# privefl/bigsnpr

Measured on NVIDIA H100. Metric: genotypes/sec in bed_prodVec, higher is better.
Workload: dtype f64

## Files before the change

bigsnpr_b200/csrc/bsg_pmv.cu:

```cuda
#include <algorithm>
#include <math.h>
#include <stdio.h>
#include <stdlib.h>
#include <string.h>

#include <cub/device/device_scan.cuh>

#include "bsg_internal.cuh"
#include "bsg_pmv_shared.cuh"

namespace bsg {
namespace pmv {

constexpr int SEG = 128;
constexpr int CODES = 512;
constexpr int DIG = 4096;
constexpr int STAGES = 6;
constexpr int STAGE_BYTES = 2 * DIG;
constexpr int SMEM_BYTES = STAGES * STAGE_BYTES + 128;
constexpr int MAX_CHUNKS_PER_ITEM = 512;

struct Args {
  const uint8_t *P;
  int64_t stride;
  const int *lines;
  int nlines;
  int nlines_pad;
  int nchunks;
  int chunks_per_split;
  int ksplit;
  const uint8_t *dig1;
  const uint8_t *dig2;
  const uint8_t *na_flags;
  int use_na;
  long long *part;
};

struct Slot {
  uint4 alo, ahi, blo, bhi;
};

__device__ __forceinline__ void slot_load(Slot &s, const uint8_t *pa, const uint8_t *pb, int64_t off) {
  s.alo = ldg_stream(pa + off);
  s.ahi = ldg_stream(pa + off + 64);
  s.blo = ldg_stream(pb + off);
  s.bhi = ldg_stream(pb + off + 64);
}

template <int MODE>
__device__ __forceinline__ uint32_t plane2(uint32_t x) {
  return MODE == 3 ? (x >> 1) : (x & (x >> 1));
}

template <int MODE, bool PRE>
__device__ __forceinline__ void chunk_mma(const Slot &t0, const Slot &t1, uint32_t dig_addr, int (&acc1)[2][4],
                                          int (&acc16)[2][4], int (&accn1)[2][4], int (&accn16)[2][4]) {
  const uint32_t wA0[8] = {t0.alo.x, t0.alo.y, t0.alo.z, t0.alo.w, t0.ahi.x, t0.ahi.y, t0.ahi.z, t0.ahi.w};
  const uint32_t wB0[8] = {t0.blo.x, t0.blo.y, t0.blo.z, t0.blo.w, t0.bhi.x, t0.bhi.y, t0.bhi.z, t0.bhi.w};
  const uint32_t wA1[8] = {t1.alo.x, t1.alo.y, t1.alo.z, t1.alo.w, t1.ahi.x, t1.ahi.y, t1.ahi.z, t1.ahi.w};
  const uint32_t wB1[8] = {t1.blo.x, t1.blo.y, t1.blo.z, t1.blo.w, t1.bhi.x, t1.bhi.y, t1.bhi.z, t1.bhi.w};
  uint4 dpre[8];
  if (PRE) {
#pragma unroll
    for (int w = 0; w < 8; w++) dpre[w] = lds128(dig_addr + w * 512);
  }
#pragma unroll
  for (int w = 0; w < 8; w++) {
    const uint4 d = PRE ? dpre[w] : lds128(dig_addr + w * 512);
    const uint32_t a0 = wA0[w], b0 = wB0[w], a1 = wA1[w], b1 = wB1[w];
    const uint32_t a0t = a0 >> 2, b0t = b0 >> 2, a1t = a1 >> 2, b1t = b1 >> 2;
    mma_u8s8(acc1[0], a0 & 0x03030303u, b0 & 0x03030303u, a0t & 0x03030303u, b0t & 0x03030303u, d.x, d.y);
    mma_u8s8(acc1[1], a1 & 0x03030303u, b1 & 0x03030303u, a1t & 0x03030303u, b1t & 0x03030303u, d.x, d.y);
    mma_u8s8(acc16[0], a0 & 0x30303030u, b0 & 0x30303030u, a0t & 0x30303030u, b0t & 0x30303030u, d.z, d.w);
    mma_u8s8(acc16[1], a1 & 0x30303030u, b1 & 0x30303030u, a1t & 0x30303030u, b1t & 0x30303030u, d.z, d.w);
    if (MODE != 0) {
      uint4 dn = d;
      if (MODE >= 2) dn = lds128(dig_addr + DIG + w * 512);
      const uint32_t a0n = plane2<MODE>(a0), b0n = plane2<MODE>(b0), a0nt = plane2<MODE>(a0t), b0nt = plane2<MODE>(b0t);
      const uint32_t a1n = plane2<MODE>(a1), b1n = plane2<MODE>(b1), a1nt = plane2<MODE>(a1t), b1nt = plane2<MODE>(b1t);
      mma_u8s8(accn1[0], a0n & 0x01010101u, b0n & 0x01010101u, a0nt & 0x01010101u, b0nt & 0x01010101u, dn.x, dn.y);
      mma_u8s8(accn1[1], a1n & 0x01010101u, b1n & 0x01010101u, a1nt & 0x01010101u, b1nt & 0x01010101u, dn.x, dn.y);
      mma_u8s8(accn16[0], a0n & 0x10101010u, b0n & 0x10101010u, a0nt & 0x10101010u, b0nt & 0x10101010u, dn.z, dn.w);
      mma_u8s8(accn16[1], a1n & 0x10101010u, b1n & 0x10101010u, a1nt & 0x10101010u, b1nt & 0x10101010u, dn.z, dn.w);
    }
  }
}

template <int MODE>
__device__ __forceinline__ void tile_mma(const Slot &sl, const uint4 (&b1)[8], uint32_t dig2_addr, int (&acc1)[4],
                                         int (&acc16)[4], int (&accn1)[4], int (&accn16)[4]) {
  const uint32_t wA[8] = {sl.alo.x, sl.alo.y, sl.alo.z, sl.alo.w, sl.ahi.x, sl.ahi.y, sl.ahi.z, sl.ahi.w};
  const uint32_t wB[8] = {sl.blo.x, sl.blo.y, sl.blo.z, sl.blo.w, sl.bhi.x, sl.bhi.y, sl.bhi.z, sl.bhi.w};
#pragma unroll
  for (int w = 0; w < 8; w++) {
    const uint32_t a = wA[w], bq = wB[w];
    const uint32_t at = a >> 2, bt = bq >> 2;
    mma_u8s8(acc1, a & 0x03030303u, bq & 0x03030303u, at & 0x03030303u, bt & 0x03030303u, b1[w].x, b1[w].y);
    mma_u8s8(acc16, a & 0x30303030u, bq & 0x30303030u, at & 0x30303030u, bt & 0x30303030u, b1[w].z, b1[w].w);
    if (MODE != 0) {
      uint4 d = b1[w];
      if (MODE >= 2) d = lds128(dig2_addr + w * 512);
      const uint32_t an = plane2<MODE>(a), bn = plane2<MODE>(bq);
      const uint32_t ant = plane2<MODE>(at), bnt = plane2<MODE>(bt);
      mma_u8s8(accn1, an & 0x01010101u, bn & 0x01010101u, ant & 0x01010101u, bnt & 0x01010101u, d.x, d.y);
      mma_u8s8(accn16, an & 0x10101010u, bn & 0x10101010u, ant & 0x10101010u, bnt & 0x10101010u, d.z, d.w);
    }
  }
}

template <int MODE, int CW, int R, int STRUCT>
__global__ void __launch_bounds__((CW + 1) * 32, 1) k_pmv(const Args a) {
  constexpr int GROUP = CW * 32;
  extern __shared__ __align__(128) uint8_t smem[];
  const int warp = threadIdx.x >> 5, lane = threadIdx.x & 31;
  const uint32_t smem_base = smem_u32(smem);
  const uint32_t bar_base = smem_base + STAGES * STAGE_BYTES;

  if (threadIdx.x == 0) {
    for (int s = 0; s < STAGES; s++) {
      mbar_init(bar_base + 8 * s, 1);
      mbar_init(bar_base + 8 * (STAGES + s), CW);
    }
    asm volatile("fence.mbarrier_init.release.cluster;" ::: "memory");
  }
  __syncthreads();

  const int ngroups = a.nlines_pad / GROUP;
  const int nitems = ngroups * a.ksplit;
  constexpr bool two_dig = MODE >= 2;
  const uint32_t stage_tx = DIG + (two_dig ? DIG : 0);

  int stage = 0;
  uint32_t phase = 0;

  if (warp == CW) {
    if (lane == 0) {
      for (int item = blockIdx.x; item < nitems; item += gridDim.x) {
        const int group = item / a.ksplit, ks = item - group * a.ksplit;
        const int c0 = ks * a.chunks_per_split;
        const int c1 = min(a.nchunks, c0 + a.chunks_per_split);
        for (int c = c0; c < c1; c++) {
          const uint32_t full = bar_base + 8 * stage, empty = bar_base + 8 * (STAGES + stage);
          mbar_wait(empty, phase ^ 1);
          mbar_expect_tx(full, stage_tx);
          const uint32_t dst = smem_base + stage * STAGE_BYTES;
          bulk_g2s(dst, a.dig1 + (int64_t)c * DIG, DIG, full);
          if (two_dig) bulk_g2s(dst + DIG, a.dig2 + (int64_t)c * DIG, DIG, full);
          if (++stage == STAGES) {
            stage = 0;
            phase ^= 1;
          }
        }
      }
    }
  } else {
    const int g = lane >> 2, q = lane & 3;
    for (int item = blockIdx.x; item < nitems; item += gridDim.x) {
      const int group = item / a.ksplit, ks = item - group * a.ksplit;
      const int c0 = ks * a.chunks_per_split;
      const int c1 = min(a.nchunks, c0 + a.chunks_per_split);
      const uint8_t *pA[2], *pB[2];
#pragma unroll
      for (int u = 0; u < 2; u++) {
        int la = min(group * GROUP + warp * 32 + u * 16 + g, a.nlines - 1);
        int lb = min(group * GROUP + warp * 32 + u * 16 + g + 8, a.nlines - 1);
        const int pa = a.lines ? a.lines[la] : la, pb = a.lines ? a.lines[lb] : lb;
        pA[u] = a.P + (int64_t)pa * a.stride + 16 * q;
        pB[u] = a.P + (int64_t)pb * a.stride + 16 * q;
      }
      bool tile_na = false;
      if (MODE == 3) {
        tile_na = true;
      } else if (MODE != 0) {
        if (a.na_flags) {
          int l = min(group * GROUP + warp * 32 + lane, a.nlines - 1);
          const int phys = a.lines ? a.lines[l] : l;
          tile_na = __any_sync(0xffffffffu, a.na_flags[phys] != 0);
        } else {
          tile_na = true;
        }
      }
      int acc1[2][4], acc16[2][4], accn1[2][4], accn16[2][4];
#pragma unroll
      for (int u = 0; u < 2; u++)
#pragma unroll
        for (int k = 0; k < 4; k++) acc1[u][k] = acc16[u][k] = accn1[u][k] = accn16[u][k] = 0;

      Slot ring[R][2];
#pragma unroll
      for (int k = 0; k < R; k++) {
        ring[k][0] = ring[k][1] =
            Slot{make_uint4(0, 0, 0, 0), make_uint4(0, 0, 0, 0), make_uint4(0, 0, 0, 0), make_uint4(0, 0, 0, 0)};
        if (c0 + k < c1) {
          slot_load(ring[k][0], pA[0], pB[0], (int64_t)(c0 + k) * SEG);
          slot_load(ring[k][1], pA[1], pB[1], (int64_t)(c0 + k) * SEG);
        }
      }

      for (int c = c0; c < c1; c += R) {
#pragma unroll
        for (int par = 0; par < R; par++) {
          if (par > 0 && c + par >= c1) break;
          const uint32_t full = bar_base + 8 * stage, empty = bar_base + 8 * (STAGES + stage);
          mbar_wait(full, phase);
          const uint32_t dbase = smem_base + stage * STAGE_BYTES + (g * 4 + q) * 16;
          const int64_t next = (int64_t)(c + par + R) * SEG;
          const bool more = (c + par + R) < c1;
          if (STRUCT == 0) {
            uint4 b1[8];
#pragma unroll
            for (int w = 0; w < 8; w++) b1[w] = lds128(dbase + w * 512);
#pragma unroll
            for (int u = 0; u < 2; u++) {
              if (MODE != 0 && tile_na)
                tile_mma<MODE>(ring[par][u], b1, dbase + DIG, acc1[u], acc16[u], accn1[u], accn16[u]);
              else
                tile_mma<0>(ring[par][u], b1, 0, acc1[u], acc16[u], accn1[u], accn16[u]);
              if (more) slot_load(ring[par][u], pA[u], pB[u], next);
            }
          } else {
            if (MODE != 0 && tile_na)
              chunk_mma<MODE, STRUCT == 2>(ring[par][0], ring[par][1], dbase, acc1, acc16, accn1, accn16);
            else
              chunk_mma<0, STRUCT == 2>(ring[par][0], ring[par][1], dbase, acc1, acc16, accn1, accn16);
            if (more) {
              slot_load(ring[par][0], pA[0], pB[0], next);
              slot_load(ring[par][1], pA[1], pB[1], next);
            }
          }
          __syncwarp();
          if (lane == 0) mbar_arrive(empty);
          if (++stage == STAGES) {
            stage = 0;
            phase ^= 1;
          }
        }
      }
#pragma unroll
      for (int u = 0; u < 2; u++) {
#pragma unroll
        for (int hrow = 0; hrow < 2; hrow++) {
          const int row = group * GROUP + warp * 32 + u * 16 + g + 8 * hrow;
          unsigned long long *dst = reinterpret_cast<unsigned long long *>(a.part) + (int64_t)row * 16 + 2 * q;
          long long vx = (long long)acc1[u][2 * hrow] + (long long)(acc16[u][2 * hrow] >> 4);
          long long vy = (long long)acc1[u][2 * hrow + 1] + (long long)(acc16[u][2 * hrow + 1] >> 4);
          atomicAdd(dst, (unsigned long long)vx);
          atomicAdd(dst + 1, (unsigned long long)vy);
          if (MODE != 0) {
            long long nx = (long long)accn1[u][2 * hrow] + (long long)(accn16[u][2 * hrow] >> 4);
            long long ny = (long long)accn1[u][2 * hrow + 1] + (long long)(accn16[u][2 * hrow + 1] >> 4);
            atomicAdd(dst + 8, (unsigned long long)nx);
            atomicAdd(dst + 9, (unsigned long long)ny);
          }
        }
      }
    }
  }
}


__device__ __forceinline__ void make_vals(int mode, const double *x, const double *center, const double *scale, int k,
                                          double &v0, double &v1) {
  if (mode == 0) {
    v0 = x[k];
    v1 = 0;
  } else if (mode == 2) {
    v0 = x[k];
    v1 = center[k];
  } else {
    double z = x[k] / scale[k];
    v0 = z;
    v1 = (center[k] - 3.0) * z;
  }
}

__global__ void k_prep1(int mode, const double *__restrict__ x, const double *__restrict__ center,
                        const double *__restrict__ scale, int len, int hb, Scal *sc) {
  __shared__ double sh[32];
  double m0 = 0, m1 = 0, cz = 0;
  int bad = 0;
  for (int k = blockIdx.x * blockDim.x + threadIdx.x; k < len; k += gridDim.x * blockDim.x) {
    double v0, v1;
    make_vals(mode, x, center, scale, k, v0, v1);
    if (!isfinite(v0) || !isfinite(v1)) bad = 1;
    m0 = fmax(m0, fabs(v0));
    m1 = fmax(m1, fabs(v1));
    if (mode == 1) cz += center[k] * v0;
  }
#pragma unroll
  for (int o = 16; o; o >>= 1) {
    m0 = fmax(m0, __shfl_xor_sync(0xffffffffu, m0, o));
    m1 = fmax(m1, __shfl_xor_sync(0xffffffffu, m1, o));
    bad |= __shfl_xor_sync(0xffffffffu, bad, o);
    cz += __shfl_xor_sync(0xffffffffu, cz, o);
  }
  if ((threadIdx.x & 31) == 0) {
    atomicMax(reinterpret_cast<unsigned long long *>(&sc->maxabs[0]), (unsigned long long)__double_as_longlong(m0));
    atomicMax(reinterpret_cast<unsigned long long *>(&sc->maxabs[1]), (unsigned long long)__double_as_longlong(m1));
    if (bad) atomicOr(&sc->nonfinite, 1);
    sh[threadIdx.x >> 5] = cz;
  }
  __syncthreads();
  if (threadIdx.x == 0) {
    double t = 0;
    for (int w = 0; w < (int)(blockDim.x >> 5); w++) t += sh[w];
    sc->cpart[blockIdx.x] = t;
    if (blockIdx.x == 0) sc->hb = hb;
  }
}

__global__ void k_quantise(int mode, const double *__restrict__ x, const double *__restrict__ center,
                           const double *__restrict__ scale, int len, const int *__restrict__ idx, const Scal *sc, int bits,
                           long long *__restrict__ Q0, long long *__restrict__ Q1) {
  const int e0 = pick_e(sc->maxabs[0], sc->hb, bits), e1 = pick_e(sc->maxabs[1], sc->hb, bits);
  const bool bad = sc->nonfinite != 0;
  for (int k = blockIdx.x * blockDim.x + threadIdx.x; k < len; k += gridDim.x * blockDim.x) {
    double v0, v1;
    make_vals(mode, x, center, scale, k, v0, v1);
    const long long q0 = bad ? 0 : __double2ll_rn(scalbn(v0, e0));
    const int t = idx ? idx[k] : k;
    atomicAdd(reinterpret_cast<unsigned long long *>(Q0 + t), (unsigned long long)q0);
    if (Q1) {
      const long long q1 = bad ? 0 : __double2ll_rn(scalbn(v1, e1));
      atomicAdd(reinterpret_cast<unsigned long long *>(Q1 + t), (unsigned long long)q1);
    }
  }
}

template <int NV>
__global__ void k_prep2(int mode, const double *__restrict__ x, const double *__restrict__ center,
                        const double *__restrict__ scale, const double *__restrict__ xb, int len, int nchunks, Scal *sc,
                        const long long *__restrict__ Q0, const long long *__restrict__ Q1, uint8_t *__restrict__ dig1,
                        uint8_t *__restrict__ dig2, int want_sum, long long *__restrict__ qout) {
  constexpr int NS = 8 / NV, BITS = NV == 1 ? 60 : 30;
  const Scal &sa = sc[0], &sb = sc[NV - 1];
  const int ea = pick_e(sa.maxabs[0], sa.hb, BITS), eb = pick_e(sb.maxabs[NV == 1 ? 1 : 0], sb.hb, BITS);
  const bool bada = sa.nonfinite != 0, badb = sb.nonfinite != 0;
  if (blockIdx.x == 0 && threadIdx.x == 0) {
    for (int v = 0; v < NV; v++) {
      sc[v].e[0] = pick_e(sc[v].maxabs[0], sc[v].hb, BITS);
      sc[v].e[1] = pick_e(sc[v].maxabs[1], sc[v].hb, BITS);
    }
  }
  long long hi = 0, lo = 0;
  const bool fasta = ea > -1000 && ea < 1000, fastb = eb > -1000 && eb < 1000;
  const double fa = fasta ? scalbn(1.0, ea) : 0.0, fb = fastb ? scalbn(1.0, eb) : 0.0;
  int64_t total = (int64_t)nchunks * 32;
  for (int64_t t = blockIdx.x * (int64_t)blockDim.x + threadIdx.x; t < total; t += (int64_t)gridDim.x * blockDim.x) {
    const int chunk = (int)(t >> 5), wq = (int)(t & 31);
    const int q = wq & 3, w = wq >> 2;
    uint32_t o1[8][4], o2[8][4];
#pragma unroll
    for (int sl = 0; sl < 8; sl++)
#pragma unroll
      for (int c = 0; c < 4; c++) o1[sl][c] = o2[sl][c] = 0;
#pragma unroll
    for (int c = 0; c < 4; c++) {
#pragma unroll
      for (int r = 0; r < 4; r++) {
        int64_t k = (int64_t)chunk * CODES + (w < 4 ? 64 * q + 16 * w : 256 + 64 * q + 16 * (w - 4)) + 4 * r + c;
        long long qa = 0, qb = 0;
        if (k < len) {
          if (Q0) {
            qa = Q0[k];
            if (Q1) qb = Q1[k];
          } else {
            double v0, v1;
            if (!bada) {
              make_vals(mode, x, center, scale, (int)k, v0, v1);
              qa = __double2ll_rn(fasta ? v0 * fa : scalbn(v0, ea));
              if (NV == 1 && dig2) qb = __double2ll_rn(fastb ? v1 * fb : scalbn(v1, eb));
            }
            if (NV == 2 && xb && !badb) {
              make_vals(mode, xb, center, scale, (int)k, v0, v1);
              qb = __double2ll_rn(fastb ? v0 * fb : scalbn(v0, eb));
            }
          }
        }
        if (want_sum) {
          hi += qa >> 32;
          lo += (long long)(unsigned int)(qa & 0xFFFFFFFFll);
        }
        if (qout && k < len) qout[k] = qa;
#pragma unroll
        for (int sl = 0; sl < NS; sl++) {
          o1[sl][c] |= (uint32_t)(peel(qa) & 0xFF) << (8 * r);
          if (NV == 2)
            o1[NS + sl][c] |= (uint32_t)(peel(qb) & 0xFF) << (8 * r);
          else if (dig2)
            o2[sl][c] |= (uint32_t)(peel(qb) & 0xFF) << (8 * r);
        }
      }
    }
#pragma unroll
    for (int sl = 0; sl < 8; sl++) {
      const int64_t unit = (int64_t)chunk * 256 + (w * 8 + sl) * 4 + q;
      reinterpret_cast<uint4 *>(dig1)[unit] = make_uint4(o1[sl][0], o1[sl][1], o1[sl][2], o1[sl][3]);
      if (NV == 1 && dig2) reinterpret_cast<uint4 *>(dig2)[unit] = make_uint4(o2[sl][0], o2[sl][1], o2[sl][2], o2[sl][3]);
    }
  }
  if (want_sum) {
#pragma unroll
    for (int o = 16; o; o >>= 1) {
      hi += __shfl_xor_sync(0xffffffffu, hi, o);
      lo += __shfl_xor_sync(0xffffffffu, lo, o);
    }
    if ((threadIdx.x & 31) == 0 && (hi | lo)) {
      atomicAdd(reinterpret_cast<unsigned long long *>(&sc->sum_hi), (unsigned long long)hi);
      atomicAdd(reinterpret_cast<unsigned long long *>(&sc->sum_lo), (unsigned long long)lo);
    }
  }
}

__global__ void k_finish_cprod(const long long *__restrict__ part, int nlines, const Scal *sc,
                               const double *__restrict__ center, const double *__restrict__ scale, int use_na,
                               double *__restrict__ out) {
  int j = blockIdx.x * blockDim.x + threadIdx.x;
  if (j >= nlines) return;
  if (sc->nonfinite) {
    out[j] = nan("");
    return;
  }
  const int e = sc->e[0];
  double G = combine<8>(part, j, 0, 1, use_na ? -3 : 0, e);
  double N = use_na ? combine<8>(part, j, 0, 0, 1, e) : 0.0;
  if (center) {
    const double Y = scalbn((double)sc->sum_hi, 32 - e) + scalbn((double)sc->sum_lo, -e);
    out[j] = (G - center[j] * (Y - N)) / scale[j];
  } else {
    out[j] = G;
  }
}

__global__ void k_finish_prod(const long long *__restrict__ part, int nlines, const Scal *sc, int has_scaling, int use_na,
                              double *__restrict__ full) {
  int l = blockIdx.x * blockDim.x + threadIdx.x;
  if (l >= nlines) return;
  full[l] = finish_prod_value(part, l, sc, has_scaling, use_na);
}

__global__ void k_finish_planes(const long long *__restrict__ part, int nlines, const Scal *sc, int have_p, int p_same,
                                double cR, double cP, double add0, double *__restrict__ full, double cRb, double cPb,
                                double *__restrict__ fullB) {
  int l = blockIdx.x * blockDim.x + threadIdx.x;
  if (l >= nlines) return;
  if (sc->nonfinite) {
    full[l] = nan("");
    if (fullB) fullB[l] = nan("");
    return;
  }
  const double R = combine<8>(part, l, 0, 1, 0, sc->e[0]);
  const double P = have_p ? combine<8>(part, l, 0, 0, 1, sc->e[p_same ? 0 : 1]) : 0.0;
  full[l] = (cR * R + cP * P) + add0;
  if (fullB) fullB[l] = cRb * R + cPb * P;
}

__global__ void k_gather(const double *__restrict__ full, const int *__restrict__ idx, int len, double *__restrict__ out) {
  int i = blockIdx.x * blockDim.x + threadIdx.x;
  if (i < len) out[i] = full[idx[i]];
}

constexpr int EV_POOL = 128;
static cudaEvent_t g_ev0[EV_POOL], g_ev1[EV_POOL];
static bool g_ev_ready = false;
static bool g_timing = false;
static int g_ev_n = 0;

static int launch_cap(int64_t work, int block, int cap) {
  int64_t g = (work + block - 1) / block;
  if (g < 1) g = 1;
  if (g > cap) g = cap;
  return (int)g;
}

static int launch_cap_pub_impl(int64_t work) { return launch_cap(work, 256, 132 * 16); }

static int hb_bits(int maxmult) {
  int b = 0;
  while ((1 << b) < maxmult) b++;
  return b >= 8 ? b + 1 : b;
}

static int prep_pmv(bsg_view *v, int dir, int mode, const double *x, const double *p1, const double *p2, int nv,
                    const double *xb, bool two, bool want_sum, bool keep_q, cudaStream_t s) {
  bsg_bed *h = v->h;
  const bool cols = dir == 0;
  const int L = cols ? h->m : h->n, len = cols ? v->nc : v->nr;
  const int *idx = (cols ? v->col_identity : v->row_identity) ? nullptr : (cols ? v->d_col : v->d_row);
  const int hb = hb_bits(cols ? v->col_maxmult : v->row_maxmult);
  const int nchunks = (int)((cols ? h->strideB : h->strideA) / SEG);
  Scal *sc = v->s_scal.as<Scal>();
  BSG_TRY(v->s_dig1.ensure((size_t)nchunks * DIG));
  if (two) BSG_TRY(v->s_dig2.ensure((size_t)nchunks * DIG));
  uint8_t *dig1 = v->s_dig1.as<uint8_t>(), *dig2 = two ? v->s_dig2.as<uint8_t>() : nullptr;
  long long *Q0 = nullptr, *Q1 = nullptr;
  if (idx || keep_q) {
    BSG_TRY(v->s_q0.ensure((size_t)L * sizeof(long long)));
    Q0 = v->s_q0.as<long long>();
  }
  if (idx && (two || xb)) {
    BSG_TRY(v->s_q1.ensure((size_t)L * sizeof(long long)));
    Q1 = v->s_q1.as<long long>();
  }
  BSG_CUDA(cudaMemsetAsync(sc, 0, nv * sizeof(Scal), s));
  k_prep1<<<SUMCZ_BLOCKS, 256, 0, s>>>(mode, x, p1, p2, len, hb, sc);
  if (xb) k_prep1<<<SUMCZ_BLOCKS, 256, 0, s>>>(mode, xb, p1, p2, len, hb, sc + 1);
  count_launch(xb ? 2 : 1);
  if (idx) {
    const int bits = nv == 1 ? 60 : 30;
    BSG_CUDA(cudaMemsetAsync(Q0, 0, (size_t)L * sizeof(long long), s));
    if (Q1) BSG_CUDA(cudaMemsetAsync(Q1, 0, (size_t)L * sizeof(long long), s));
    k_quantise<<<launch_cap(len, 256, 592), 256, 0, s>>>(mode, x, p1, p2, len, idx, sc, bits, Q0, nv == 1 ? Q1 : nullptr);
    if (xb) k_quantise<<<launch_cap(len, 256, 592), 256, 0, s>>>(mode, xb, p1, p2, len, idx, sc + 1, bits, Q1, nullptr);
    count_launch(xb ? 2 : 1);
  }
  const int grid = launch_cap((int64_t)nchunks * 32, 128, 1184);
  const long long *src0 = idx ? Q0 : nullptr;
  if (nv == 1)
    k_prep2<1><<<grid, 128, 0, s>>>(mode, x, p1, p2, nullptr, L, nchunks, sc, src0, Q1, dig1, dig2, want_sum,
                                    idx ? nullptr : Q0);
  else
    k_prep2<2><<<grid, 128, 0, s>>>(mode, x, p1, p2, xb, L, nchunks, sc, src0, Q1, dig1, nullptr, want_sum, nullptr);
  count_launch();
  return BSG_OK;
}

static int run_pmv(bsg_view *v, const uint8_t *P, int64_t stride, int L, const int *lines, int nlines,
                   const uint8_t *dig1, const uint8_t *dig2, const uint8_t *na_flags, int use_na, Args *out_args,
                   cudaStream_t s, bool plane_hi = false) {
  static int var_cw = 0, var_r = 0, var_s = 0;
  if (!var_cw) {
    var_cw = 11;
    var_r = 3;
    var_s = 1;
    const char *ev = getenv("BSG_PMV_VARIANT");
    int cw = 0, r = 0, st = 0;
    if (ev && sscanf(ev, "%dx%ds%d", &cw, &r, &st) >= 2) {
      if ((cw == 11 || cw == 15) && (r == 2 || r == 3) && st >= 0 && st <= 2) {
        var_cw = cw;
        var_r = r;
        var_s = st;
      }
    }
  }
  const int GROUP = var_cw * 32;
  Args a;
  a.P = P;
  a.stride = stride;
  a.lines = lines;
  a.nlines = nlines;
  a.nlines_pad = (int)round_up(nlines, GROUP);
  a.nchunks = (int)(round_up(((int64_t)L + 3) / 4, SEG) / SEG);
  int ngroups = a.nlines_pad / GROUP;
  int target_items = 24 * 132;
  int ks = (target_items + ngroups - 1) / ngroups;
  int ks_max = std::max(1, a.nchunks / 16);
  int ks_min = (a.nchunks + MAX_CHUNKS_PER_ITEM - 1) / MAX_CHUNKS_PER_ITEM;
  ks = std::min(ks, ks_max);
  ks = std::max(ks, ks_min);
  ks = std::max(ks, 1);
  a.chunks_per_split = (a.nchunks + ks - 1) / ks;
  a.ksplit = (a.nchunks + a.chunks_per_split - 1) / a.chunks_per_split;
  a.dig1 = dig1;
  a.dig2 = dig2;
  a.na_flags = na_flags;
  a.use_na = use_na;
  BSG_TRY(v->s_part.ensure((size_t)a.nlines_pad * 16 * sizeof(long long)));
  a.part = v->s_part.as<long long>();
  BSG_CUDA(cudaMemsetAsync(a.part, 0, (size_t)a.nlines_pad * 16 * sizeof(long long), s));
  const int mode = plane_hi ? 3 : (!use_na ? 0 : (dig2 ? 2 : 1));
  if (plane_hi && !dig2) return fail(BSG_ERR_ARG, "high-bit plane needs its own digits");
  void (*kern)(const Args) = nullptr;
#define PMV_PICK(CWv, Rv, Sv)                                                                   \
  if (var_cw == CWv && var_r == Rv && var_s == Sv)                                              \
    kern = mode == 0 ? k_pmv<0, CWv, Rv, Sv>                                                    \
                     : (mode == 1 ? k_pmv<1, CWv, Rv, Sv> : (mode == 2 ? k_pmv<2, CWv, Rv, Sv> : k_pmv<3, CWv, Rv, Sv>));
  PMV_PICK(11, 2, 0)
  PMV_PICK(11, 2, 1)
  PMV_PICK(11, 2, 2)
  PMV_PICK(11, 3, 0)
  PMV_PICK(11, 3, 1)
  PMV_PICK(15, 2, 1)
#undef PMV_PICK
  if (!kern) return fail(BSG_ERR_ARG, "unknown k_pmv variant");
  BSG_CUDA(cudaFuncSetAttribute(kern, cudaFuncAttributeMaxDynamicSharedMemorySize, SMEM_BYTES));
  int nsm = 132;
  cudaDeviceGetAttribute(&nsm, cudaDevAttrMultiProcessorCount, v->h->device);
  int nitems = ngroups * a.ksplit;
  int grid = std::min(nitems, nsm);
  if (g_timing) cudaEventRecord(g_ev0[g_ev_n % EV_POOL], s);
  kern<<<grid, (var_cw + 1) * 32, SMEM_BYTES, s>>>(a);
  if (g_timing) {
    cudaEventRecord(g_ev1[g_ev_n % EV_POOL], s);
    g_ev_n++;
  }
  count_launch();
  BSG_CUDA(cudaGetLastError());
  *out_args = a;
  return BSG_OK;
}

}

namespace pmvt {
using namespace pmv;
constexpr int TLINES = 32, TBYTES = 512, TWARPS = 8, TSTAGES = 6;
constexpr int WSTAGE_BYTES = TLINES * 64;
constexpr int TSMEM = TWARPS * TSTAGES * WSTAGE_BYTES;
constexpr int MAX_LINES_PER_ITEM = 1 << 16;

struct TArgs {
  const uint8_t *P;
  int64_t stride;
  const int *lines;
  int nlines;
  const uint8_t *dig;
  int lines_per_split, ksplit, nblocks, n;
  long long *part;
};

__device__ __forceinline__ void cp_async16(uint32_t dst, const void *src, int src_bytes) {
  asm volatile("cp.async.cg.shared.global [%0], [%1], 16, %2;" ::"r"(dst), "l"(src), "r"(src_bytes) : "memory");
}

template <int PLANE>
__global__ void __launch_bounds__(TWARPS * 32, 2) k_pmvT_lines(const TArgs a) {
  extern __shared__ __align__(128) uint8_t smem[];
  const int tid = threadIdx.x, warp = tid >> 5, lane = tid & 31, g = lane >> 2, q = lane & 3;
  const int blk = blockIdx.x % a.nblocks, ks = blockIdx.x / a.nblocks;
  const int64_t byte0 = (int64_t)blk * TBYTES + 64 * warp;
  const int l0 = ks * a.lines_per_split, l1 = min(a.nlines, l0 + a.lines_per_split);
  const int nsteps = (l1 - l0 + TLINES - 1) / TLINES;
  const uint32_t wbase = smem_u32(smem) + warp * (TSTAGES * WSTAGE_BYTES);

  const int lrow = lane >> 2, lch = lane & 3;
  const int64_t colb = (byte0 + 16 * lch < a.stride) ? byte0 + 16 * lch : 0;
  uint32_t dst_off[4];
#pragma unroll
  for (int i = 0; i < 4; i++) {
    const int row = 8 * i + lrow;
    const int hf = row >> 4, qq = (row >> 2) & 3, r = row & 3, sl = lch >> 1, hc = lch & 1;
    dst_off[i] = (uint32_t)((((((r * 2 + hf) * 2 + sl) * 4 + qq) * 8) + 4 * hc) * 4);
  }
  auto issue = [&](int step, int stage) {
    const uint32_t dst = wbase + stage * WSTAGE_BYTES;
#pragma unroll
    for (int i = 0; i < 4; i++) {
      const int t = min(l0 + step * TLINES + 8 * i + lrow, l1 - 1);
      const int phys = a.lines[t];
      cp_async16(dst + dst_off[i], a.P + colb + (int64_t)phys * a.stride, 16);
    }
  };

  int acc[4][4][4];
#pragma unroll
  for (int j = 0; j < 4; j++)
#pragma unroll
    for (int c = 0; c < 4; c++)
#pragma unroll
      for (int k = 0; k < 4; k++) acc[j][c][k] = 0;

#pragma unroll
  for (int st = 0; st < TSTAGES - 1; st++) {
    if (st < nsteps) issue(st, st);
    asm volatile("cp.async.commit_group;" ::: "memory");
  }
  const uint8_t *dg = a.dig + (int64_t)(l0 / TLINES) * 256 + g * 32 + 4 * q;
  uint32_t nb0 = 0, nb1 = 0;
  if (nsteps > 0) {
    nb0 = *reinterpret_cast<const uint32_t *>(dg);
    nb1 = *reinterpret_cast<const uint32_t *>(dg + 16);
  }
  const uint32_t rd_base = wbase + (uint32_t)((q * 8 + g) * 4);

  auto compute = [&](uint32_t st_base, uint32_t b0, uint32_t b1) {
    uint32_t W[2][2][4];
#pragma unroll
    for (int sl = 0; sl < 2; sl++)
#pragma unroll
      for (int hf = 0; hf < 2; hf++) {
        const uint32_t ad = st_base + (hf * 2 + sl) * 128;
        const uint32_t x0 = lds32(ad), x1 = lds32(ad + 512), x2 = lds32(ad + 1024), x3 = lds32(ad + 1536);
        const uint32_t t0 = prmt(x0, x1, 0x5140), t1 = prmt(x2, x3, 0x5140);
        const uint32_t t2 = prmt(x0, x1, 0x7362), t3 = prmt(x2, x3, 0x7362);
        W[sl][hf][0] = prmt(t0, t1, 0x5410);
        W[sl][hf][1] = prmt(t0, t1, 0x7632);
        W[sl][hf][2] = prmt(t2, t3, 0x5410);
        W[sl][hf][3] = prmt(t2, t3, 0x7632);
      }
#pragma unroll
    for (int j = 0; j < 4; j++) {
      uint32_t wa = W[0][0][j], wb = W[1][0][j], wc2 = W[0][1][j], wd = W[1][1][j];
      if (PLANE == 1) {
        wa = wa & (wa >> 1) & 0x55555555u;
        wb = wb & (wb >> 1) & 0x55555555u;
        wc2 = wc2 & (wc2 >> 1) & 0x55555555u;
        wd = wd & (wd >> 1) & 0x55555555u;
      } else if (PLANE == 2) {
        wa = (wa >> 1) & 0x55555555u;
        wb = (wb >> 1) & 0x55555555u;
        wc2 = (wc2 >> 1) & 0x55555555u;
        wd = (wd >> 1) & 0x55555555u;
      }
      mma_u8s8(acc[j][0], wa & 0x03030303u, wb & 0x03030303u, wc2 & 0x03030303u, wd & 0x03030303u, b0, b1);
      mma_u8s8(acc[j][1], wa & 0x0C0C0C0Cu, wb & 0x0C0C0C0Cu, wc2 & 0x0C0C0C0Cu, wd & 0x0C0C0C0Cu, b0, b1);
      mma_u8s8(acc[j][2], wa & 0x30303030u, wb & 0x30303030u, wc2 & 0x30303030u, wd & 0x30303030u, b0, b1);
      mma_u8s8(acc[j][3], wa & 0xC0C0C0C0u, wb & 0xC0C0C0C0u, wc2 & 0xC0C0C0C0u, wd & 0xC0C0C0C0u, b0, b1);
    }
  };

  uint32_t rd_stage = 0, wr_stage = (TSTAGES - 1) * WSTAGE_BYTES;
  const uint8_t *dgn = dg + 256;
  for (int step = 0; step < nsteps; step++) {
    asm volatile("cp.async.wait_group %0;" ::"n"(TSTAGES - 2) : "memory");
    __syncwarp();
    {
      const int nxt = step + TSTAGES - 1;
      if (nxt < nsteps) issue(nxt, (int)(wr_stage / WSTAGE_BYTES));
      asm volatile("cp.async.commit_group;" ::: "memory");
    }
    const uint32_t b0 = nb0, b1 = nb1;
    if (step + 1 < nsteps) {
      nb0 = *reinterpret_cast<const uint32_t *>(dgn);
      nb1 = *reinterpret_cast<const uint32_t *>(dgn + 16);
      dgn += 256;
    }
    compute(rd_base + rd_stage, b0, b1);
    rd_stage = rd_stage + WSTAGE_BYTES == TSTAGES * WSTAGE_BYTES ? 0 : rd_stage + WSTAGE_BYTES;
    wr_stage = wr_stage + WSTAGE_BYTES == TSTAGES * WSTAGE_BYTES ? 0 : wr_stage + WSTAGE_BYTES;
  }
  asm volatile("cp.async.wait_group 0;" ::: "memory");
#pragma unroll
  for (int j = 0; j < 4; j++)
#pragma unroll
    for (int c = 0; c < 4; c++)
#pragma unroll
      for (int sl = 0; sl < 2; sl++) {
        const int64_t sample = 4 * (byte0 + 4 * (8 * sl + g) + j) + c;
        if (sample < a.n) {
          unsigned long long *dst = reinterpret_cast<unsigned long long *>(a.part) + sample * 16 + (PLANE ? 8 : 0) + 2 * q;
          long long v0 = acc[j][c][2 * sl], v1 = acc[j][c][2 * sl + 1];
          v0 >>= 2 * c;
          v1 >>= 2 * c;
          if (v0) atomicAdd(dst, (unsigned long long)v0);
          if (v1) atomicAdd(dst + 1, (unsigned long long)v1);
        }
      }
}

constexpr int TBOX = 32 * 128;
constexpr int TDIG_OFF = 4 * TBOX;
constexpr int TSTAGE_BYTES = 4 * TBOX + 1024;
constexpr int TCSTAGES = 6;
constexpr int TSMEM_TMA = TCSTAGES * TSTAGE_BYTES + 2 * TCSTAGES * 8 + 1024;


template <int PLANE>
__global__ void __launch_bounds__(TWARPS * 32, 2) k_pmvT(const __grid_constant__ CUtensorMap map, const TArgs a) {
  extern __shared__ __align__(128) uint8_t smem[];
  const int tid = threadIdx.x, warp = tid >> 5, lane = tid & 31, g = lane >> 2, q = lane & 3;
  const int blk = blockIdx.x % a.nblocks, ks = blockIdx.x / a.nblocks;
  const int l0 = ks * a.lines_per_split, l1 = min(a.nlines, l0 + a.lines_per_split);
  const int nsteps = (l1 - l0 + TLINES - 1) / TLINES;
  const uint32_t sbase = (smem_u32(smem) + 1023u) & ~1023u;
  const uint32_t bar_base = sbase + TCSTAGES * TSTAGE_BYTES;
  auto fill = [&](int step, int st) {
    const uint32_t full = bar_base + 8 * st, dst = sbase + st * TSTAGE_BYTES;
    const uint8_t *dg = a.dig + (int64_t)(l0 / TLINES + step) * 256;
    mbar_expect_tx(full, 4 * TBOX + 256);
#pragma unroll
    for (int j = 0; j < 4; j++) tma_load_2d(dst + j * TBOX, &map, full, blk * TBYTES + 128 * j, l0 + step * TLINES);
    bulk_g2s(dst + TDIG_OFF, dg, 128, full);
    bulk_g2s(dst + TDIG_OFF + 144, dg + 128, 128, full);
  };
  if (tid == 0) {
    for (int st = 0; st < TCSTAGES; st++) {
      mbar_init(bar_base + 8 * st, 1);
      mbar_init(bar_base + 8 * (TCSTAGES + st), TWARPS);
    }
    asm volatile("fence.mbarrier_init.release.cluster;" ::: "memory");
    for (int st = 0; st < min(TCSTAGES, nsteps); st++) fill(st, st);
  }
  __syncthreads();
  int stage = 0, pstage = 0;
  uint32_t phase = 0, pphase = 0;

  const int64_t byte0 = (int64_t)blk * TBYTES + 64 * warp;
  const int rsw = 2 * (q >> 1);
  const uint32_t chunk0 = (4 * (warp & 1) + (g >> 2)) ^ (4 * (q & 1) + rsw);
  const uint32_t rd_base = sbase + (warp >> 1) * TBOX + q * 512 + (rsw << 7) + chunk0 * 16 + 4 * (g & 3);
  const uint32_t dg_base = sbase + TDIG_OFF + g * 32 + 16 * (g >> 2) + 4 * q;
  const uint32_t sel_lo = rsw ? 0x1054u : 0x5410u, sel_hi = rsw ? 0x3276u : 0x7632u;

  int acc[4][4][4];
#pragma unroll
  for (int j = 0; j < 4; j++)
#pragma unroll
    for (int c = 0; c < 4; c++)
#pragma unroll
      for (int k = 0; k < 4; k++) acc[j][c][k] = 0;

  for (int step = 0; step < nsteps; step++) {
    const uint32_t full = bar_base + 8 * stage, empty = bar_base + 8 * (TCSTAGES + stage);
    const uint32_t so = stage * TSTAGE_BYTES;
    const int cstage = stage;
    const uint32_t cphase = phase;
    mbar_wait(full, phase);
    const uint32_t b0 = lds32(dg_base + so), b1 = lds32(dg_base + so + 16);
    uint32_t W[2][2][4];
#pragma unroll
    for (int sl = 0; sl < 2; sl++)
#pragma unroll
      for (int hf = 0; hf < 2; hf++) {
        const uint32_t ad = rd_base + so, hb = hf * (16 * 128);
        const uint32_t x0 = lds32((ad ^ TRD(0, sl)) + hb), x1 = lds32((ad ^ TRD(1, sl)) + hb);
        const uint32_t x2 = lds32((ad ^ TRD(2, sl)) + hb), x3 = lds32((ad ^ TRD(3, sl)) + hb);
        const uint32_t t0 = prmt(x0, x1, 0x5140), t1 = prmt(x2, x3, 0x5140);
        const uint32_t t2 = prmt(x0, x1, 0x7362), t3 = prmt(x2, x3, 0x7362);
        W[sl][hf][0] = prmt(t0, t1, sel_lo);
        W[sl][hf][1] = prmt(t0, t1, sel_hi);
        W[sl][hf][2] = prmt(t2, t3, sel_lo);
        W[sl][hf][3] = prmt(t2, t3, sel_hi);
      }
    __syncwarp();
    if (lane == 0) mbar_arrive(empty);
    if (++stage == TCSTAGES) {
      stage = 0;
      phase ^= 1;
    }
#pragma unroll
    for (int j = 0; j < 4; j++) {
      uint32_t wa = W[0][0][j], wb = W[1][0][j], wc2 = W[0][1][j], wd = W[1][1][j];
      if (PLANE == 1) {
        wa = wa & (wa >> 1) & 0x55555555u;
        wb = wb & (wb >> 1) & 0x55555555u;
        wc2 = wc2 & (wc2 >> 1) & 0x55555555u;
        wd = wd & (wd >> 1) & 0x55555555u;
      } else if (PLANE == 2) {
        wa = (wa >> 1) & 0x55555555u;
        wb = (wb >> 1) & 0x55555555u;
        wc2 = (wc2 >> 1) & 0x55555555u;
        wd = (wd >> 1) & 0x55555555u;
      }
      mma_u8s8(acc[j][0], wa & 0x03030303u, wb & 0x03030303u, wc2 & 0x03030303u, wd & 0x03030303u, b0, b1);
      mma_u8s8(acc[j][1], wa & 0x0C0C0C0Cu, wb & 0x0C0C0C0Cu, wc2 & 0x0C0C0C0Cu, wd & 0x0C0C0C0Cu, b0, b1);
      mma_u8s8(acc[j][2], wa & 0x30303030u, wb & 0x30303030u, wc2 & 0x30303030u, wd & 0x30303030u, b0, b1);
      mma_u8s8(acc[j][3], wa & 0xC0C0C0C0u, wb & 0xC0C0C0C0u, wc2 & 0xC0C0C0C0u, wd & 0xC0C0C0C0u, b0, b1);
    }
    if (tid == 0 && step >= 1 && step - 1 + TCSTAGES < nsteps) {
      mbar_wait(bar_base + 8 * (TCSTAGES + pstage), pphase);
      fill(step - 1 + TCSTAGES, pstage);
    }
    __syncwarp();
    pstage = cstage;
    pphase = cphase;
  }
#pragma unroll
  for (int j = 0; j < 4; j++)
#pragma unroll
    for (int c = 0; c < 4; c++)
#pragma unroll
      for (int sl = 0; sl < 2; sl++) {
        const int64_t sample = 4 * (byte0 + 4 * (8 * sl + g) + j) + c;
        if (sample < a.n) {
          unsigned long long *dst = reinterpret_cast<unsigned long long *>(a.part) + sample * 16 + (PLANE ? 8 : 0) + 2 * q;
          long long v0 = acc[j][c][2 * sl], v1 = acc[j][c][2 * sl + 1];
          v0 >>= 2 * c;
          v1 >>= 2 * c;
          if (v0) atomicAdd(dst, (unsigned long long)v0);
          if (v1) atomicAdd(dst + 1, (unsigned long long)v1);
        }
      }
}

constexpr int W2STAGE_BYTES = TLINES * 32;
constexpr int T2BYTES = TWARPS * 32;
constexpr int T2SMEM = TWARPS * TSTAGES * W2STAGE_BYTES;

template <int PL, bool LINES>
__global__ void __launch_bounds__(TWARPS * 32, 2) k_pmvT2(const TArgs a, const uint8_t *__restrict__ dig2) {
  extern __shared__ __align__(128) uint8_t smem[];
  const int tid = threadIdx.x, warp = tid >> 5, lane = tid & 31, g = lane >> 2, q = lane & 3;
  const int blk = blockIdx.x % a.nblocks, ks = blockIdx.x / a.nblocks;
  const int64_t byte0 = (int64_t)blk * T2BYTES + 32 * warp;
  const int l0 = ks * a.lines_per_split, l1 = min(a.nlines, l0 + a.lines_per_split);
  const int nsteps = (l1 - l0 + TLINES - 1) / TLINES;
  const uint32_t wbase = smem_u32(smem) + warp * (TSTAGES * W2STAGE_BYTES);
  const int lrow = lane >> 1, lch = lane & 1;
  const int64_t colb = (byte0 + 16 * lch < a.stride) ? byte0 + 16 * lch : 0;
  uint32_t dst_off[2];
// ... 1296 lines not shown
```

Measured before the change: 11640 billion.

## Add per-line L2 bulk prefetch and cost-based k-split selection to pmv kernel

Each compute thread issues cp.async.bulk.prefetch.L2 for its genotype row, first for the leading chunks of its split and then four chunks ahead every four chunks, so that DRAM latency is hidden behind the register ring loads. The host also chooses chunks_per_split as a multiple of four, using a cost model over wave count and chunk count. This variant is the default. It adds extra prefetch instructions and can change load balance across SMs, and the new sscanf pattern means variant strings without a p field leave pf at 0.

```diff
diff --git a/bigsnpr_b200/csrc/bsg_pmv.cu b/bigsnpr_b200/csrc/bsg_pmv.cu
--- a/bigsnpr_b200/csrc/bsg_pmv.cu
+++ b/bigsnpr_b200/csrc/bsg_pmv.cu
@@ -45,6 +45,10 @@
   s.ahi = ldg_stream(pa + off + 64);
   s.blo = ldg_stream(pb + off);
   s.bhi = ldg_stream(pb + off + 64);
+}
+
+__device__ __forceinline__ void prefetch_l2(const uint8_t *p, uint32_t bytes) {
+  asm volatile("cp.async.bulk.prefetch.L2.global [%0], %1;" ::"l"(p), "r"(bytes) : "memory");
 }
 
 template <int MODE>
@@ -108,7 +112,7 @@
   }
 }
 
-template <int MODE, int CW, int R, int STRUCT>
+template <int MODE, int CW, int R, int STRUCT, bool PF>
 __global__ void __launch_bounds__((CW + 1) * 32, 1) k_pmv(const Args a) {
   constexpr int GROUP = CW * 32;
   extern __shared__ __align__(128) uint8_t smem[];
@@ -168,6 +172,12 @@
         pA[u] = a.P + (int64_t)pa * a.stride + 16 * q;
         pB[u] = a.P + (int64_t)pb * a.stride + 16 * q;
       }
+      const uint8_t *pL = nullptr;
+      if (PF) {
+        const int l = min(group * GROUP + warp * 32 + lane, a.nlines - 1);
+        pL = a.P + (int64_t)(a.lines ? a.lines[l] : l) * a.stride;
+        prefetch_l2(pL + (int64_t)c0 * SEG, (uint32_t)min(8, c1 - c0) * SEG);
+      }
       bool tile_na = false;
       if (MODE == 3) {
         tile_na = true;
@@ -206,6 +216,11 @@
           const uint32_t dbase = smem_base + stage * STAGE_BYTES + (g * 4 + q) * 16;
           const int64_t next = (int64_t)(c + par + R) * SEG;
           const bool more = (c + par + R) < c1;
+          if (PF) {
+            const int cc = c + par;
+            if (cc > c0 && ((cc - c0) & 3) == 0 && cc + 4 < c1)
+              prefetch_l2(pL + (int64_t)(cc + 4) * SEG, (uint32_t)min(4, c1 - cc - 4) * SEG);
+          }
           if (STRUCT == 0) {
             uint4 b1[8];
 #pragma unroll
@@ -528,18 +543,20 @@
 static int run_pmv(bsg_view *v, const uint8_t *P, int64_t stride, int L, const int *lines, int nlines,
                    const uint8_t *dig1, const uint8_t *dig2, const uint8_t *na_flags, int use_na, Args *out_args,
                    cudaStream_t s, bool plane_hi = false) {
-  static int var_cw = 0, var_r = 0, var_s = 0;
+  static int var_cw = 0, var_r = 0, var_s = 0, var_pf = 0;
   if (!var_cw) {
     var_cw = 11;
     var_r = 3;
     var_s = 1;
+    var_pf = 1;
     const char *ev = getenv("BSG_PMV_VARIANT");
-    int cw = 0, r = 0, st = 0;
-    if (ev && sscanf(ev, "%dx%ds%d", &cw, &r, &st) >= 2) {
-      if ((cw == 11 || cw == 15) && (r == 2 || r == 3) && st >= 0 && st <= 2) {
+    int cw = 0, r = 0, st = 0, pf = 0;
+    if (ev && sscanf(ev, "%dx%ds%dp%d", &cw, &r, &st, &pf) >= 2) {
+      if ((cw == 11 || cw == 15) && (r == 2 || r == 3) && st >= 0 && st <= 2 && (pf == 0 || pf == 1)) {
         var_cw = cw;
         var_r = r;
         var_s = st;
+        var_pf = pf;
       }
     }
   }
@@ -552,6 +569,8 @@
   a.nlines_pad = (int)round_up(nlines, GROUP);
   a.nchunks = (int)(round_up(((int64_t)L + 3) / 4, SEG) / SEG);
   int ngroups = a.nlines_pad / GROUP;
+  int nsm = 132;
+  cudaDeviceGetAttribute(&nsm, cudaDevAttrMultiProcessorCount, v->h->device);
   int target_items = 24 * 132;
   int ks = (target_items + ngroups - 1) / ngroups;
   int ks_max = std::max(1, a.nchunks / 16);
@@ -559,7 +578,19 @@
   ks = std::min(ks, ks_max);
   ks = std::max(ks, ks_min);
   ks = std::max(ks, 1);
-  a.chunks_per_split = (a.nchunks + ks - 1) / ks;
+  if (!var_pf) {
+    a.chunks_per_split = (a.nchunks + ks - 1) / ks;
+  } else {
+    auto cps_of = [&](int k) { return (int)round_up((a.nchunks + k - 1) / k, 4); };
+    auto cost = [&](int k) {
+      const int cps = cps_of(k), kk = (a.nchunks + cps - 1) / cps;
+      return (int64_t)((ngroups * kk + nsm - 1) / nsm) * (cps + 4);
+    };
+    int best = ks;
+    for (int k = ks + 1; k <= std::min(2 * ks, ks_max); k++)
+      if (cps_of(k) <= MAX_CHUNKS_PER_ITEM && cost(k) < cost(best)) best = k;
+    a.chunks_per_split = std::min(cps_of(best), MAX_CHUNKS_PER_ITEM);
+  }
   a.ksplit = (a.nchunks + a.chunks_per_split - 1) / a.chunks_per_split;
   a.dig1 = dig1;
   a.dig2 = dig2;
@@ -571,21 +602,21 @@
   const int mode = plane_hi ? 3 : (!use_na ? 0 : (dig2 ? 2 : 1));
   if (plane_hi && !dig2) return fail(BSG_ERR_ARG, "high-bit plane needs its own digits");
   void (*kern)(const Args) = nullptr;
-#define PMV_PICK(CWv, Rv, Sv)                                                                   \
-  if (var_cw == CWv && var_r == Rv && var_s == Sv)                                              \
-    kern = mode == 0 ? k_pmv<0, CWv, Rv, Sv>                                                    \
-                     : (mode == 1 ? k_pmv<1, CWv, Rv, Sv> : (mode == 2 ? k_pmv<2, CWv, Rv, Sv> : k_pmv<3, CWv, Rv, Sv>));
-  PMV_PICK(11, 2, 0)
-  PMV_PICK(11, 2, 1)
-  PMV_PICK(11, 2, 2)
-  PMV_PICK(11, 3, 0)
-  PMV_PICK(11, 3, 1)
-  PMV_PICK(15, 2, 1)
+#define PMV_PICK(CWv, Rv, Sv, PFv)                                                                  \
+  if (var_cw == CWv && var_r == Rv && var_s == Sv && var_pf == PFv)                                 \
+    kern = mode == 0 ? k_pmv<0, CWv, Rv, Sv, PFv>                                                   \
+                     : (mode == 1 ? k_pmv<1, CWv, Rv, Sv, PFv>                                      \
+                                  : (mode == 2 ? k_pmv<2, CWv, Rv, Sv, PFv> : k_pmv<3, CWv, Rv, Sv, PFv>));
+  PMV_PICK(11, 2, 0, false)
+  PMV_PICK(11, 2, 1, false)
+  PMV_PICK(11, 2, 2, false)
+  PMV_PICK(11, 3, 0, false)
+  PMV_PICK(11, 3, 1, false)
+  PMV_PICK(15, 2, 1, false)
+  PMV_PICK(11, 3, 1, true)
 #undef PMV_PICK
   if (!kern) return fail(BSG_ERR_ARG, "unknown k_pmv variant");
   BSG_CUDA(cudaFuncSetAttribute(kern, cudaFuncAttributeMaxDynamicSharedMemorySize, SMEM_BYTES));
-  int nsm = 132;
-  cudaDeviceGetAttribute(&nsm, cudaDevAttrMultiProcessorCount, v->h->device);
   int nitems = ngroups * a.ksplit;
   int grid = std::min(nitems, nsm);
   if (g_timing) cudaEventRecord(g_ev0[g_ev_n % EV_POOL], s);
```

Result: no change. 11640 billion (median of 6 runs) (+0.0%).
